# krasserm/perceiver-io

Hardware: NVIDIA H100
Metric: cross_attn_core_tflops (higher is better)
Workload: dtype bf16

## Files before the change

### perceiver_io_b200/csrc/pcv_kvproj.cu

```cuda
#include "pcv_common.cuh"
#include "pcv_sm90.cuh"

#include <algorithm>
#include <cstdlib>

namespace pcv {
namespace {

using namespace sm90;

constexpr int kBM = 128;
constexpr int kBN = 128;
constexpr int kBK = 64;
constexpr int kGemmThreads = 384;
constexpr int kStages = 6;
constexpr int kBoxBytes = 128 * 128;
constexpr int kStageBytes = 2 * kBoxBytes;
constexpr int kSmemBytes = kStages * kStageBytes + 2048 + 1024;

struct GemmParams {
  const float2* stats;
  const float2* col_st;
  void* k_out;
  void* v_out;
  const void* x;
  int64_t x_stride, k_stride, v_stride;
  int64_t rows;
  int n_k, n_total;
  int num_kb;
  int tiles_n;
  int C;
  float eps;
};

struct Fp8Out {
  const float* inv_scale;
  void* vt_out;
  int64_t vt_sb, vt_sh, vt_sc;
  int64_t keys_per_batch;
  int v_dv;
};

struct GemmSmem {
  uint64_t full[kStages], empty[kStages];
  float2 row_st[kBM];
};

template <bool BF16, bool FUSE, int CG, bool F8>
__device__ __forceinline__ void kvproj_body(const CUtensorMap& tx, const CUtensorMap& tw, const GemmParams& p,
                                            const Fp8Out& f8) {
  static_assert(!F8 || CG == 1, "the e4m3 producer runs one CTA per tile");
  using T = typename std::conditional<BF16, __nv_bfloat16, __half>::type;
  extern __shared__ __align__(1024) uint8_t smem_raw[];
  uint8_t* smem = reinterpret_cast<uint8_t*>((reinterpret_cast<uintptr_t>(smem_raw) + 1023) & ~uintptr_t(1023));
  GemmSmem& sh = *reinterpret_cast<GemmSmem*>(smem + kStages * kStageBytes);
  const int wg = threadIdx.x / 128;
  const uint32_t rank = CG == 2 ? cluster_ctarank() : 0u;
  const int64_t cid = blockIdx.x / CG;
  const int n_blk = (int)(cid % p.tiles_n);
  const int64_t m_blk = (cid / p.tiles_n) * CG + rank;
  const int64_t row0 = m_blk * kBM;
  const int col0 = n_blk * kBN;

  if (threadIdx.x == 0) {
    for (int s = 0; s < kStages; ++s) {
      mbar_init(&sh.full[s], 1);
      mbar_init(&sh.empty[s], CG == 2 ? 16 : 8);
    }
    fence_mbar_init();
  }
  if (CG == 2)
    cluster_sync_all();
  else
    __syncthreads();

  if (wg == 0) {
    reg_dealloc<40>();
    if (threadIdx.x == 0) {
      for (int kb = 0; kb < p.num_kb; ++kb) {
// ... 7 lines not shown
        else
          tma_load_2d(smem + s * kStageBytes + kBoxBytes, &tw, &sh.full[s], kb * kBK, col0);
      }
    }
    if (CG == 2) {
      __syncwarp();
      cluster_sync_all();
    }
    return;
  }

  reg_alloc<232>();
  const int cw = wg - 1;
  const int tid = threadIdx.x - 128 * wg;
  const int warp = tid >> 5, lane = tid & 31;
  const int rloc = 64 * cw + 16 * warp + (lane >> 2);
  const int cq = 2 * (lane & 3);
  const uint32_t base = smem_u32(smem);
  const int srow = 64 * cw + (tid >> 1), shalf = tid & 1;
  float x0 = 0.f, s1 = 0.f, s2 = 0.f;
  if (FUSE && row0 + srow < p.rows)
    x0 = Elem<T>::to_f(*(reinterpret_cast<const T*>(p.x) + (row0 + srow) * p.x_stride));

  float acc[64];
  for (int kb = 0; kb < p.num_kb; ++kb) {
    const int s = kb % kStages;
    mbar_wait(&sh.full[s], (kb / kStages) & 1, 12);
    wgmma_fence();
#pragma unroll
    for (int kk = 0; kk < 4; ++kk)
      wgmma_ss<128, BF16>(acc, make_desc(base + s * kStageBytes + cw * 64 * 128 + kk * 32),
                          make_desc(base + s * kStageBytes + kBoxBytes + kk * 32), (kb | kk) != 0);
    wgmma_commit();
    if (FUSE) {
      const uint8_t* line = smem + s * kStageBytes + srow * 128;
#pragma unroll
      for (int ch = 0; ch < 4; ++ch) {
        const int lc = shalf * 4 + ch;
        const uint4 u = *reinterpret_cast<const uint4*>(line + ((lc ^ (srow & 7)) * 16));
        const typename Elem<T>::T2* h2 = reinterpret_cast<const typename Elem<T>::T2*>(&u);
#pragma unroll
        for (int e = 0; e < 4; ++e) {
          const int c = kb * kBK + lc * 8 + 2 * e;
          const float2 f = Elem<T>::to_f2(h2[e]);
          if (c < p.C) {
            const float d = f.x - x0;
            s1 += d;
            s2 = fmaf(d, d, s2);
          }
          if (c + 1 < p.C) {
            const float d = f.y - x0;
            s1 += d;
            s2 = fmaf(d, d, s2);
          }
        }
      }
    }
    wgmma_wait<0>();
    fence_regs(acc);
    if (CG == 2) warp_arrive_pair(&sh.empty[s]);
    else warp_arrive(&sh.empty[s]);
  }

  if (FUSE) {
    s1 += __shfl_xor_sync(0xffffffffu, s1, 1);
    s2 += __shfl_xor_sync(0xffffffffu, s2, 1);
    if (shalf == 0) {
      const float inv_c = 1.f / (float)p.C;
      const float dm = s1 * inv_c;
      const float var = fmaxf(s2 * inv_c - dm * dm, 0.f);
      sh.row_st[srow] = make_float2(x0 + dm, var > 0.f ? rsqrtf(var + p.eps) : 0.f);
    }
    asm volatile("bar.sync %0, 128;" ::"r"(1 + cw) : "memory");
  }

  const float rstd_flat = p.eps > 0.f ? 1.f / sqrtf(p.eps) : -1.f;
#pragma unroll
  for (int r = 0; r < 2; ++r) {
    const int64_t row = row0 + rloc + 8 * r;
    if (row >= p.rows) continue;
    float2 st = make_float2(0.f, 1.f);
    const bool ln = FUSE || p.stats != nullptr;
    if (FUSE) {
      st = sh.row_st[rloc + 8 * r];
    } else if (p.stats != nullptr) {
      st = p.stats[row];
      if (st.y == rstd_flat) st.y = 0.f;
    }
#pragma unroll
    for (int g = 0; g < 16; ++g) {
      const int n = col0 + 8 * g + cq;
      if (n >= p.n_total) continue;
      const float2 c0 = p.col_st[n], c1 = p.col_st[n + 1];
      float a0 = acc[4 * g + 2 * r], a1 = acc[4 * g + 2 * r + 1];
      if (ln) {
        a0 = st.y * (a0 - st.x * c0.x);
        a1 = st.y * (a1 - st.x * c1.x);
      }
      if constexpr (F8) {
        const uint32_t w8 = cvt_e4m3x2((a0 + c0.y) * f8.inv_scale[n], (a1 + c1.y) * f8.inv_scale[n + 1]);
        if (n < p.n_k) {
          *reinterpret_cast<uint16_t*>(reinterpret_cast<uint8_t*>(p.k_out) + row * p.k_stride + n) = (uint16_t)w8;
        } else {
          const int c = n - p.n_k, h = c / f8.v_dv;
          const int64_t b = row / f8.keys_per_batch, m = row - b * f8.keys_per_batch;
          uint8_t* dst = reinterpret_cast<uint8_t*>(f8.vt_out) + b * f8.vt_sb + h * f8.vt_sh +
                         (int64_t)(c - h * f8.v_dv) * f8.vt_sc + m;
          dst[0] = (uint8_t)(w8 & 0xffu);
          dst[f8.vt_sc] = (uint8_t)(w8 >> 8);
        }
      } else {
        const uint32_t w = pack2(a0 + c0.y, a1 + c1.y, BF16);
        if (n < p.n_k)
          *reinterpret_cast<uint32_t*>(reinterpret_cast<T*>(p.k_out) + row * p.k_stride + n) = w;
        else
          *reinterpret_cast<uint32_t*>(reinterpret_cast<T*>(p.v_out) + row * p.v_stride + (n - p.n_k)) = w;
      }
    }
  }
  if (CG == 2) cluster_sync_all();
}

template <bool BF16, bool FUSE, int CG>
__global__ void __launch_bounds__(kGemmThreads, 1)
kvproj_kernel(const __grid_constant__ CUtensorMap tx, const __grid_constant__ CUtensorMap tw, const GemmParams p) {
  kvproj_body<BF16, FUSE, CG, false>(tx, tw, p, Fp8Out{});
}

template <bool BF16, bool FUSE>
__global__ void __launch_bounds__(kGemmThreads, 1)
kvproj_fp8_kernel(const __grid_constant__ CUtensorMap tx, const __grid_constant__ CUtensorMap tw, const GemmParams p,
                  const Fp8Out f8) {
  kvproj_body<BF16, FUSE, 1, true>(tx, tw, p, f8);
}


template <typename T, int NCH>
__global__ void __launch_bounds__(256) ln_stats_reg_kernel(const T* __restrict__ x, int64_t stride_row, int64_t rows,
                                                            float eps, float2* __restrict__ stats) {
  constexpr int C = NCH * 256;
  const int lane = threadIdx.x & 31;
  const int64_t warps = (int64_t)gridDim.x * (blockDim.x >> 5);
  const int64_t w0 = (int64_t)blockIdx.x * (blockDim.x >> 5) + (threadIdx.x >> 5);
  for (int64_t r = w0 * 2; r < rows; r += warps * 2) {
    uint4 u[2][NCH];
#pragma unroll
    for (int k = 0; k < 2; ++k) {
      const bool live = r + k < rows;
      const uint4* xr = reinterpret_cast<const uint4*>(x + (r + k) * stride_row);
#pragma unroll
      for (int i = 0; i < NCH; ++i) u[k][i] = live ? __ldcs(xr + lane + 32 * i) : make_uint4(0, 0, 0, 0);
    }
#pragma unroll
    for (int k = 0; k < 2; ++k) {
      float sum = 0.f;
#pragma unroll
      for (int i = 0; i < NCH; ++i) {
        const typename Elem<T>::T2* h = reinterpret_cast<const typename Elem<T>::T2*>(&u[k][i]);
#pragma unroll
        for (int j = 0; j < 4; ++j) {
          const float2 f = Elem<T>::to_f2(h[j]);
          sum += f.x + f.y;
        }
      }
      const float mean = warp_sum(sum) / (float)C;
      float sq = 0.f;
#pragma unroll
      for (int i = 0; i < NCH; ++i) {
// ... 69 lines not shown
    const int blocks = (int)std::min<int64_t>((p.rows + 15) / 16, 132 * 8);
#define PCV_LN_CASE(N)                                                                               \
  case N:                                                                                            \
    ln_stats_reg_kernel<T, N><<<blocks, 256, 0, stream>>>(x, p.x_stride_row, p.rows, p.eps, st);     \
    break;
    switch (p.C / 256) {
      PCV_LN_CASE(1) PCV_LN_CASE(2) PCV_LN_CASE(3) PCV_LN_CASE(4) PCV_LN_CASE(5) PCV_LN_CASE(6) PCV_LN_CASE(7)
      PCV_LN_CASE(8)
    }
#undef PCV_LN_CASE
  } else {
    const int blocks = (int)std::min<int64_t>((p.rows + 7) / 8, 132 * 8);
    ln_stats_kernel<T><<<blocks, 256, 0, stream>>>(x, p.x_stride_row, p.rows, p.C, p.eps, st);
  }
  PCV_CHECK_CUDA(cudaGetLastError());
  count_launch();
  return PCV_OK;
}

template <bool BF16, bool FUSE, int CG, bool F8 = false>
int launch_gemm(const CUtensorMap& tx, const CUtensorMap& tw, const GemmParams& gp, cudaStream_t stream,
                const Fp8Out& f8 = Fp8Out{}) {
  const int64_t m_blocks = (gp.rows + kBM * CG - 1) / (kBM * CG) * CG;
  const int64_t tiles = m_blocks * gp.tiles_n;
  PCV_REQUIRE(tiles <= 0x7fffffff, PCV_ERR_UNSUPPORTED, "kv_project: %lld tiles exceed the grid limit", (long long)tiles);
  prof_mark_begin(stream);
  int rc;
  if constexpr (F8)
    rc = launch_kernel(kvproj_fp8_kernel<BF16, FUSE>, dim3((unsigned)tiles), kGemmThreads, kSmemBytes, 0, stream, tx, tw,
                       gp, f8);
  else
    rc = launch_kernel(kvproj_kernel<BF16, FUSE, CG>, dim3((unsigned)tiles), kGemmThreads, kSmemBytes, CG, stream,
                       tx, tw, gp);
  prof_mark_end(stream);
  return rc;
}

}

int launch_ln_stats(const pcv_ln_stats_params& p, cudaStream_t stream) {
  PCV_REQUIRE(p.x != nullptr && p.stats != nullptr, PCV_ERR_INVALID, "ln_stats: NULL pointer");
  PCV_REQUIRE(p.rows >= 0 && p.C >= 1, PCV_ERR_INVALID, "ln_stats: rows=%lld C=%d", (long long)p.rows, p.C);
  PCV_REQUIRE(p.dtype == PCV_BF16 || p.dtype == PCV_F16, PCV_ERR_INVALID, "ln_stats: dtype must be bf16/fp16");
  if (p.rows == 0) return PCV_OK;
  return p.dtype == PCV_BF16 ? launch_ln_stats_t<__nv_bfloat16>(p, stream) : launch_ln_stats_t<__half>(p, stream);
}

bool kv_project_supported(const pcv_kvproj_params& p, const char** why) {
  auto fail = [&](const char* w) {
    *why = w;
    return false;
  };
  if (p.dtype != PCV_BF16 && p.dtype != PCV_F16) return fail("dtype must be bf16 or fp16");
  if (p.C < 8 || (p.C % 8)) return fail("input channels must be a multiple of 8 (16-byte TMA strides)");
  if (p.n_k < 0 || p.n_v < 0 || p.n_k + p.n_v < 1) return fail("no output columns");
  if ((p.n_k % 64) != 0) return fail("K width must be a multiple of 64");
  if ((p.n_v % 8) != 0) return fail("V width must be a multiple of 8");
  if (!al16(p.x) || !al16(p.w) || (p.n_k && !al16(p.k_out)) || (p.n_v && !al16(p.v_out)))
    return fail("x / w / k_out / v_out must be 16-byte aligned");
  if ((p.x_stride_row % 8) || (p.k_stride_row % 8) || (p.v_stride_row % 8)) return fail("row strides must be multiples of 8 elements");
  if (p.rows < 1 || p.rows > (int64_t)0x7fffff00) return fail("row count out of range");
  if (p.cta_group < 0 || p.cta_group > 2) return fail("cta_group must be 0, 1 or 2");
  if (const char* w = device_problem()) return fail(w);
  return true;
}

// ... 57 lines not shown
  if (fuse)
    return bf ? launch_gemm<true, true, 1, true>(tx, tw, gp, stream, f8) : launch_gemm<false, true, 1, true>(tx, tw, gp, stream, f8);
  return bf ? launch_gemm<true, false, 1, true>(tx, tw, gp, stream, f8) : launch_gemm<false, false, 1, true>(tx, tw, gp, stream, f8);
}

int launch_kv_project(const pcv_kvproj_params& p, cudaStream_t stream) {
  const char* why = "";
  PCV_REQUIRE(p.x && p.w && p.col_st, PCV_ERR_INVALID, "kv_project: NULL pointer");
  PCV_REQUIRE(kv_project_supported(p, &why), PCV_ERR_UNSUPPORTED, "kv_project: %s", why);
  const int n_total = p.n_k + p.n_v;
  GemmParams gp{};
  gp.stats = reinterpret_cast<const float2*>(p.row_stats);
  gp.col_st = reinterpret_cast<const float2*>(p.col_st);
  gp.k_out = p.k_out;
  gp.v_out = p.v_out;
  gp.x = p.x;
  gp.x_stride = p.x_stride_row;
  gp.k_stride = p.k_stride_row;
  gp.v_stride = p.v_stride_row;
  gp.rows = p.rows;
  gp.n_k = p.n_k;
  gp.n_total = n_total;
  gp.num_kb = (p.C + kBK - 1) / kBK;
  gp.tiles_n = (n_total + kBN - 1) / kBN;
  gp.C = p.C;
  gp.eps = p.ln_eps;
  const bool fuse = p.row_stats == nullptr && p.ln_eps > 0.f;

  int rc = attach_wait_diag(&g_wait_diag);
  if (rc != PCV_OK) return rc;
  CUtensorMap tx, tw;
  rc = make_tmap_2d(&tx, p.x, p.dtype, p.C, p.rows, p.x_stride_row, kBM);
  if (rc != PCV_OK) return rc;
  const int cg = p.cta_group == 2 ? 2 : 1;
  rc = make_tmap_2d(&tw, p.w, p.dtype, p.C, n_total, p.C, kBN / cg);
  if (rc != PCV_OK) return rc;
  const bool bf = p.dtype == PCV_BF16;
#define PCV_GEMM_CASE(G)                                                                                   \
  if (fuse) return bf ? launch_gemm<true, true, G>(tx, tw, gp, stream) : launch_gemm<false, true, G>(tx, tw, gp, stream); \
  return bf ? launch_gemm<true, false, G>(tx, tw, gp, stream) : launch_gemm<false, false, G>(tx, tw, gp, stream);
  if (cg == 2) {
    PCV_GEMM_CASE(2)
  }
  PCV_GEMM_CASE(1)
#undef PCV_GEMM_CASE
}

}
```

### perceiver_io_b200/csrc/pcv_sm90.cuh

```cuda
#pragma once

#include <cstdint>
#include <utility>
#include <cuda.h>
#include <cuda_runtime.h>

#include "pcv_common.cuh"

namespace pcv {
namespace sm90 {

__device__ __forceinline__ uint32_t smem_u32(const void* p) {
  return static_cast<uint32_t>(__cvta_generic_to_shared(p));
}

__device__ __forceinline__ void mbar_init(uint64_t* bar, uint32_t count) {
  asm volatile("mbarrier.init.shared::cta.b64 [%0], %1;" ::"r"(smem_u32(bar)), "r"(count) : "memory");
}
__device__ __forceinline__ void fence_mbar_init() {
  asm volatile("fence.mbarrier_init.release.cluster;" ::: "memory");
}
__device__ __forceinline__ void fence_proxy_async_smem() {
  asm volatile("fence.proxy.async.shared::cta;" ::: "memory");
}
// ... 51 lines not shown
  }
}

__device__ __forceinline__ void warp_arrive(uint64_t* bar) {
  __syncwarp();
  if ((threadIdx.x & 31) == 0) mbar_arrive(bar);
}

template <int ID, int THREADS>
__device__ __forceinline__ void named_bar_sync() {
  asm volatile("bar.sync %0, %1;" ::"n"(ID), "n"(THREADS) : "memory");
}
template <int ID, int THREADS>
__device__ __forceinline__ void named_bar_arrive() {
  asm volatile("bar.arrive %0, %1;" ::"n"(ID), "n"(THREADS) : "memory");
}

__device__ __forceinline__ void tma_load_4d(void* smem_dst, const void* tmap, uint64_t* bar, int c0, int c1,
                                            int c2, int c3) {
  asm volatile(
      "cp.async.bulk.tensor.4d.shared::cluster.global.mbarrier::complete_tx::bytes [%0], [%1, {%3, %4, %5, %6}], "
      "[%2];" ::"r"(smem_u32(smem_dst)),
      "l"(reinterpret_cast<uint64_t>(tmap)), "r"(smem_u32(bar)), "r"(c0), "r"(c1), "r"(c2), "r"(c3)
      : "memory");
}
__device__ __forceinline__ void tma_load_2d(void* smem_dst, const void* tmap, uint64_t* bar, int c0, int c1) {
  asm volatile(
      "cp.async.bulk.tensor.2d.shared::cluster.global.mbarrier::complete_tx::bytes [%0], [%1, {%3, %4}], [%2];" ::"r"(
          smem_u32(smem_dst)),
      "l"(reinterpret_cast<uint64_t>(tmap)), "r"(smem_u32(bar)), "r"(c0), "r"(c1)
      : "memory");
}

__device__ __forceinline__ uint32_t cluster_ctarank() {
  uint32_t r;
  asm volatile("mov.u32 %0, %%cluster_ctarank;" : "=r"(r));
  return r;
}
__device__ __forceinline__ void cluster_sync_all() {
  asm volatile("barrier.cluster.arrive.release.aligned;\n\tbarrier.cluster.wait.acquire.aligned;" ::: "memory");
}
__device__ __forceinline__ void mbar_arrive_cta(uint64_t* bar, uint32_t cta) {
  uint32_t remote;
  asm volatile("mapa.shared::cluster.u32 %0, %1, %2;" : "=r"(remote) : "r"(smem_u32(bar)), "r"(cta));
  asm volatile("mbarrier.arrive.release.cluster.shared::cluster.b64 _, [%0];" ::"r"(remote) : "memory");
}
__device__ __forceinline__ void warp_arrive_pair(uint64_t* bar) {
  __syncwarp();
  if ((threadIdx.x & 31) == 0) {
    mbar_arrive_cta(bar, 0);
    mbar_arrive_cta(bar, 1);
  }
}
__device__ __forceinline__ void wg_arrive(uint64_t* bar) {
  if ((threadIdx.x & 127) == 0) mbar_arrive(bar);
}
__device__ __forceinline__ void wg_arrive_pair(uint64_t* bar) {
  const uint32_t t = threadIdx.x & 127;
  if (t == 0) mbar_arrive(bar);
  else if (t == 32) mbar_arrive_cta(bar, cluster_ctarank() ^ 1u);
}
__device__ __forceinline__ void tma_load_4d_mc(void* smem_dst, const void* tmap, uint64_t* bar, int c0, int c1, int c2,
                                               int c3, uint16_t mask) {
  asm volatile(
      "cp.async.bulk.tensor.4d.shared::cluster.global.mbarrier::complete_tx::bytes.multicast::cluster [%0], [%1, {%3, "
      "%4, %5, %6}], [%2], %7;" ::"r"(smem_u32(smem_dst)),
// ... 107 lines not shown
      "{%0, %1, %2, %3, %4, %5, %6, %7, %8, %9, %10, %11, %12, %13, %14, %15, %16, %17, %18, %19, %20, %21, %22, %23, %24, %25, %26, %27, %28, %29, %30, %31, %32, %33, %34, %35, %36, %37, %38, %39, %40, %41, %42, %43, %44, %45, %46, %47, %48, %49, %50, %51, %52, %53, %54, %55, %56, %57, %58, %59, %60, %61, %62, %63}, %64, %65, p, 1, 1, 0, 0;\n\t}"
      : "+f"(d[0]), "+f"(d[1]), "+f"(d[2]), "+f"(d[3]), "+f"(d[4]), "+f"(d[5]), "+f"(d[6]), "+f"(d[7]), "+f"(d[8]), "+f"(d[9]), "+f"(d[10]), "+f"(d[11]), "+f"(d[12]), "+f"(d[13]), "+f"(d[14]), "+f"(d[15]), "+f"(d[16]), "+f"(d[17]), "+f"(d[18]), "+f"(d[19]), "+f"(d[20]), "+f"(d[21]), "+f"(d[22]), "+f"(d[23]), "+f"(d[24]), "+f"(d[25]), "+f"(d[26]), "+f"(d[27]), "+f"(d[28]), "+f"(d[29]), "+f"(d[30]), "+f"(d[31]), "+f"(d[32]), "+f"(d[33]), "+f"(d[34]), "+f"(d[35]), "+f"(d[36]), "+f"(d[37]), "+f"(d[38]), "+f"(d[39]), "+f"(d[40]), "+f"(d[41]), "+f"(d[42]), "+f"(d[43]), "+f"(d[44]), "+f"(d[45]), "+f"(d[46]), "+f"(d[47]), "+f"(d[48]), "+f"(d[49]), "+f"(d[50]), "+f"(d[51]), "+f"(d[52]), "+f"(d[53]), "+f"(d[54]), "+f"(d[55]), "+f"(d[56]), "+f"(d[57]), "+f"(d[58]), "+f"(d[59]), "+f"(d[60]), "+f"(d[61]), "+f"(d[62]), "+f"(d[63])
      : "l"(a), "l"(b), "r"(scale_d));
}

template <>
__device__ __forceinline__ void wgmma_rs<64, false>(float (&d)[32], const uint32_t (&a)[4], uint64_t b) {
  asm volatile(
      "{\n\t.reg .pred p;\n\tsetp.ne.b32 p, 1, 0;\n\t"
      "wgmma.mma_async.sync.aligned.m64n64k16.f32.f16.f16 "
      "{%0, %1, %2, %3, %4, %5, %6, %7, %8, %9, %10, %11, %12, %13, %14, %15, %16, %17, %18, %19, %20, %21, %22, %23, %24, %25, %26, %27, %28, %29, %30, %31}, {%32, %33, %34, %35}, %36, p, 1, 1, 1;\n\t}"
      : "+f"(d[0]), "+f"(d[1]), "+f"(d[2]), "+f"(d[3]), "+f"(d[4]), "+f"(d[5]), "+f"(d[6]), "+f"(d[7]), "+f"(d[8]), "+f"(d[9]), "+f"(d[10]), "+f"(d[11]), "+f"(d[12]), "+f"(d[13]), "+f"(d[14]), "+f"(d[15]), "+f"(d[16]), "+f"(d[17]), "+f"(d[18]), "+f"(d[19]), "+f"(d[20]), "+f"(d[21]), "+f"(d[22]), "+f"(d[23]), "+f"(d[24]), "+f"(d[25]), "+f"(d[26]), "+f"(d[27]), "+f"(d[28]), "+f"(d[29]), "+f"(d[30]), "+f"(d[31])
      : "r"(a[0]), "r"(a[1]), "r"(a[2]), "r"(a[3]), "l"(b));
}

template <>
__device__ __forceinline__ void wgmma_rs<128, true>(float (&d)[64], const uint32_t (&a)[4], uint64_t b) {
  asm volatile(
      "{\n\t.reg .pred p;\n\tsetp.ne.b32 p, 1, 0;\n\t"
      "wgmma.mma_async.sync.aligned.m64n128k16.f32.bf16.bf16 "
      "{%0, %1, %2, %3, %4, %5, %6, %7, %8, %9, %10, %11, %12, %13, %14, %15, %16, %17, %18, %19, %20, %21, %22, %23, %24, %25, %26, %27, %28, %29, %30, %31, %32, %33, %34, %35, %36, %37, %38, %39, %40, %41, %42, %43, %44, %45, %46, %47, %48, %49, %50, %51, %52, %53, %54, %55, %56, %57, %58, %59, %60, %61, %62, %63}, {%64, %65, %66, %67}, %68, p, 1, 1, 1;\n\t}"
      : "+f"(d[0]), "+f"(d[1]), "+f"(d[2]), "+f"(d[3]), "+f"(d[4]), "+f"(d[5]), "+f"(d[6]), "+f"(d[7]), "+f"(d[8]), "+f"(d[9]), "+f"(d[10]), "+f"(d[11]), "+f"(d[12]), "+f"(d[13]), "+f"(d[14]), "+f"(d[15]), "+f"(d[16]), "+f"(d[17]), "+f"(d[18]), "+f"(d[19]), "+f"(d[20]), "+f"(d[21]), "+f"(d[22]), "+f"(d[23]), "+f"(d[24]), "+f"(d[25]), "+f"(d[26]), "+f"(d[27]), "+f"(d[28]), "+f"(d[29]), "+f"(d[30]), "+f"(d[31]), "+f"(d[32]), "+f"(d[33]), "+f"(d[34]), "+f"(d[35]), "+f"(d[36]), "+f"(d[37]), "+f"(d[38]), "+f"(d[39]), "+f"(d[40]), "+f"(d[41]), "+f"(d[42]), "+f"(d[43]), "+f"(d[44]), "+f"(d[45]), "+f"(d[46]), "+f"(d[47]), "+f"(d[48]), "+f"(d[49]), "+f"(d[50]), "+f"(d[51]), "+f"(d[52]), "+f"(d[53]), "+f"(d[54]), "+f"(d[55]), "+f"(d[56]), "+f"(d[57]), "+f"(d[58]), "+f"(d[59]), "+f"(d[60]), "+f"(d[61]), "+f"(d[62]), "+f"(d[63])
      : "r"(a[0]), "r"(a[1]), "r"(a[2]), "r"(a[3]), "l"(b));
}

template <>
__device__ __forceinline__ void wgmma_rs<128, false>(float (&d)[64], const uint32_t (&a)[4], uint64_t b) {
  asm volatile(
      "{\n\t.reg .pred p;\n\tsetp.ne.b32 p, 1, 0;\n\t"
      "wgmma.mma_async.sync.aligned.m64n128k16.f32.f16.f16 "
      "{%0, %1, %2, %3, %4, %5, %6, %7, %8, %9, %10, %11, %12, %13, %14, %15, %16, %17, %18, %19, %20, %21, %22, %23, %24, %25, %26, %27, %28, %29, %30, %31, %32, %33, %34, %35, %36, %37, %38, %39, %40, %41, %42, %43, %44, %45, %46, %47, %48, %49, %50, %51, %52, %53, %54, %55, %56, %57, %58, %59, %60, %61, %62, %63}, {%64, %65, %66, %67}, %68, p, 1, 1, 1;\n\t}"
      : "+f"(d[0]), "+f"(d[1]), "+f"(d[2]), "+f"(d[3]), "+f"(d[4]), "+f"(d[5]), "+f"(d[6]), "+f"(d[7]), "+f"(d[8]), "+f"(d[9]), "+f"(d[10]), "+f"(d[11]), "+f"(d[12]), "+f"(d[13]), "+f"(d[14]), "+f"(d[15]), "+f"(d[16]), "+f"(d[17]), "+f"(d[18]), "+f"(d[19]), "+f"(d[20]), "+f"(d[21]), "+f"(d[22]), "+f"(d[23]), "+f"(d[24]), "+f"(d[25]), "+f"(d[26]), "+f"(d[27]), "+f"(d[28]), "+f"(d[29]), "+f"(d[30]), "+f"(d[31]), "+f"(d[32]), "+f"(d[33]), "+f"(d[34]), "+f"(d[35]), "+f"(d[36]), "+f"(d[37]), "+f"(d[38]), "+f"(d[39]), "+f"(d[40]), "+f"(d[41]), "+f"(d[42]), "+f"(d[43]), "+f"(d[44]), "+f"(d[45]), "+f"(d[46]), "+f"(d[47]), "+f"(d[48]), "+f"(d[49]), "+f"(d[50]), "+f"(d[51]), "+f"(d[52]), "+f"(d[53]), "+f"(d[54]), "+f"(d[55]), "+f"(d[56]), "+f"(d[57]), "+f"(d[58]), "+f"(d[59]), "+f"(d[60]), "+f"(d[61]), "+f"(d[62]), "+f"(d[63])
      : "r"(a[0]), "r"(a[1]), "r"(a[2]), "r"(a[3]), "l"(b));
}

template <bool BF16>
__device__ __forceinline__ void wgmma_ss_bmn_n128(float (&d)[64], uint64_t a, uint64_t b, int scale_d) {
  if constexpr (BF16)
    asm volatile(
        "{\n\t.reg .pred p;\n\tsetp.ne.b32 p, %66, 0;\n\t"
        "wgmma.mma_async.sync.aligned.m64n128k16.f32.bf16.bf16 "
        "{%0, %1, %2, %3, %4, %5, %6, %7, %8, %9, %10, %11, %12, %13, %14, %15, %16, %17, %18, %19, %20, %21, %22, %23, %24, %25, %26, %27, %28, %29, %30, %31, %32, %33, %34, %35, %36, %37, %38, %39, %40, %41, %42, %43, %44, %45, %46, %47, %48, %49, %50, %51, %52, %53, %54, %55, %56, %57, %58, %59, %60, %61, %62, %63}, %64, %65, p, 1, 1, 0, 1;\n\t}"
        : "+f"(d[0]), "+f"(d[1]), "+f"(d[2]), "+f"(d[3]), "+f"(d[4]), "+f"(d[5]), "+f"(d[6]), "+f"(d[7]), "+f"(d[8]), "+f"(d[9]), "+f"(d[10]), "+f"(d[11]), "+f"(d[12]), "+f"(d[13]), "+f"(d[14]), "+f"(d[15]), "+f"(d[16]), "+f"(d[17]), "+f"(d[18]), "+f"(d[19]), "+f"(d[20]), "+f"(d[21]), "+f"(d[22]), "+f"(d[23]), "+f"(d[24]), "+f"(d[25]), "+f"(d[26]), "+f"(d[27]), "+f"(d[28]), "+f"(d[29]), "+f"(d[30]), "+f"(d[31]), "+f"(d[32]), "+f"(d[33]), "+f"(d[34]), "+f"(d[35]), "+f"(d[36]), "+f"(d[37]), "+f"(d[38]), "+f"(d[39]), "+f"(d[40]), "+f"(d[41]), "+f"(d[42]), "+f"(d[43]), "+f"(d[44]), "+f"(d[45]), "+f"(d[46]), "+f"(d[47]), "+f"(d[48]), "+f"(d[49]), "+f"(d[50]), "+f"(d[51]), "+f"(d[52]), "+f"(d[53]), "+f"(d[54]), "+f"(d[55]), "+f"(d[56]), "+f"(d[57]), "+f"(d[58]), "+f"(d[59]), "+f"(d[60]), "+f"(d[61]), "+f"(d[62]), "+f"(d[63])
        : "l"(a), "l"(b), "r"(scale_d));
  else
    asm volatile(
        "{\n\t.reg .pred p;\n\tsetp.ne.b32 p, %66, 0;\n\t"
        "wgmma.mma_async.sync.aligned.m64n128k16.f32.f16.f16 "
        "{%0, %1, %2, %3, %4, %5, %6, %7, %8, %9, %10, %11, %12, %13, %14, %15, %16, %17, %18, %19, %20, %21, %22, %23, %24, %25, %26, %27, %28, %29, %30, %31, %32, %33, %34, %35, %36, %37, %38, %39, %40, %41, %42, %43, %44, %45, %46, %47, %48, %49, %50, %51, %52, %53, %54, %55, %56, %57, %58, %59, %60, %61, %62, %63}, %64, %65, p, 1, 1, 0, 1;\n\t}"
        : "+f"(d[0]), "+f"(d[1]), "+f"(d[2]), "+f"(d[3]), "+f"(d[4]), "+f"(d[5]), "+f"(d[6]), "+f"(d[7]), "+f"(d[8]), "+f"(d[9]), "+f"(d[10]), "+f"(d[11]), "+f"(d[12]), "+f"(d[13]), "+f"(d[14]), "+f"(d[15]), "+f"(d[16]), "+f"(d[17]), "+f"(d[18]), "+f"(d[19]), "+f"(d[20]), "+f"(d[21]), "+f"(d[22]), "+f"(d[23]), "+f"(d[24]), "+f"(d[25]), "+f"(d[26]), "+f"(d[27]), "+f"(d[28]), "+f"(d[29]), "+f"(d[30]), "+f"(d[31]), "+f"(d[32]), "+f"(d[33]), "+f"(d[34]), "+f"(d[35]), "+f"(d[36]), "+f"(d[37]), "+f"(d[38]), "+f"(d[39]), "+f"(d[40]), "+f"(d[41]), "+f"(d[42]), "+f"(d[43]), "+f"(d[44]), "+f"(d[45]), "+f"(d[46]), "+f"(d[47]), "+f"(d[48]), "+f"(d[49]), "+f"(d[50]), "+f"(d[51]), "+f"(d[52]), "+f"(d[53]), "+f"(d[54]), "+f"(d[55]), "+f"(d[56]), "+f"(d[57]), "+f"(d[58]), "+f"(d[59]), "+f"(d[60]), "+f"(d[61]), "+f"(d[62]), "+f"(d[63])
        : "l"(a), "l"(b), "r"(scale_d));
}

__device__ __forceinline__ void ldsm_x4_trans(uint32_t (&r)[4], uint32_t addr) {
  asm volatile("ldmatrix.sync.aligned.m8n8.x4.trans.shared.b16 {%0, %1, %2, %3}, [%4];"
               : "=r"(r[0]), "=r"(r[1]), "=r"(r[2]), "=r"(r[3])
               : "r"(addr)
               : "memory");
}

__device__ __forceinline__ void wgmma_ss_e4m3_n128(float (&d)[64], uint64_t a, uint64_t b, int scale_d) {
  asm volatile(
      "{\n\t.reg .pred p;\n\tsetp.ne.b32 p, %66, 0;\n\t"
      "wgmma.mma_async.sync.aligned.m64n128k32.f32.e4m3.e4m3 "
      "{%0, %1, %2, %3, %4, %5, %6, %7, %8, %9, %10, %11, %12, %13, %14, %15, %16, %17, %18, %19, %20, %21, %22, %23, %24, %25, %26, %27, %28, %29, %30, %31, %32, %33, %34, %35, %36, %37, %38, %39, %40, %41, %42, %43, %44, %45, %46, %47, %48, %49, %50, %51, %52, %53, %54, %55, %56, %57, %58, %59, %60, %61, %62, %63}, %64, %65, p, 1, 1;\n\t}"
      : "+f"(d[0]), "+f"(d[1]), "+f"(d[2]), "+f"(d[3]), "+f"(d[4]), "+f"(d[5]), "+f"(d[6]), "+f"(d[7]), "+f"(d[8]), "+f"(d[9]), "+f"(d[10]), "+f"(d[11]), "+f"(d[12]), "+f"(d[13]), "+f"(d[14]), "+f"(d[15]), "+f"(d[16]), "+f"(d[17]), "+f"(d[18]), "+f"(d[19]), "+f"(d[20]), "+f"(d[21]), "+f"(d[22]), "+f"(d[23]), "+f"(d[24]), "+f"(d[25]), "+f"(d[26]), "+f"(d[27]), "+f"(d[28]), "+f"(d[29]), "+f"(d[30]), "+f"(d[31]), "+f"(d[32]), "+f"(d[33]), "+f"(d[34]), "+f"(d[35]), "+f"(d[36]), "+f"(d[37]), "+f"(d[38]), "+f"(d[39]), "+f"(d[40]), "+f"(d[41]), "+f"(d[42]), "+f"(d[43]), "+f"(d[44]), "+f"(d[45]), "+f"(d[46]), "+f"(d[47]), "+f"(d[48]), "+f"(d[49]), "+f"(d[50]), "+f"(d[51]), "+f"(d[52]), "+f"(d[53]), "+f"(d[54]), "+f"(d[55]), "+f"(d[56]), "+f"(d[57]), "+f"(d[58]), "+f"(d[59]), "+f"(d[60]), "+f"(d[61]), "+f"(d[62]), "+f"(d[63])
// ... 48 lines not shown
```

Measured before the change: 589.9.

## Add persistent 128x256 KV-projection GEMM with TMA-store epilogue

Adds a persistent warp-specialized kernel, used when cta_group is 0 and there are at least as many tiles as SMs. It uses 128x256 tiles with m64n256 wgmma and keeps one wgmma group in flight across k-blocks. Output goes through swizzled shared-memory staging and TMA bulk stores, aiming to cut launch and tail overhead and to overlap the epilogue with the next tile's loads. In exchange it uses 128 fp32 accumulators per thread, has only 3 pipeline stages, and does not handle the fp8 path. The workload metric is cross-attention core TFLOPS, so the kv-projection may not dominate it.

```diff
diff --git a/perceiver_io_b200/csrc/pcv_kvproj.cu b/perceiver_io_b200/csrc/pcv_kvproj.cu
--- a/perceiver_io_b200/csrc/pcv_kvproj.cu
+++ b/perceiver_io_b200/csrc/pcv_kvproj.cu
@@ -45,6 +45,64 @@
   uint64_t full[kStages], empty[kStages];
   float2 row_st[kBM];
 };
+
+template <typename T>
+__device__ __forceinline__ void stats_accumulate(const uint8_t* line, int srow, int shalf, int kb, const GemmParams& p,
+                                                 float x0, float& s1, float& s2) {
+#pragma unroll
+  for (int ch = 0; ch < 4; ++ch) {
+    const int lc = shalf * 4 + ch;
+    const uint4 u = *reinterpret_cast<const uint4*>(line + ((lc ^ (srow & 7)) * 16));
+    const typename Elem<T>::T2* h2 = reinterpret_cast<const typename Elem<T>::T2*>(&u);
+#pragma unroll
+    for (int e = 0; e < 4; ++e) {
+      const int c = kb * kBK + lc * 8 + 2 * e;
+      const float2 f = Elem<T>::to_f2(h2[e]);
+      if (c < p.C) {
+        const float d = f.x - x0;
+        s1 += d;
+        s2 = fmaf(d, d, s2);
+      }
+      if (c + 1 < p.C) {
+        const float d = f.y - x0;
+        s1 += d;
+        s2 = fmaf(d, d, s2);
+      }
+    }
+  }
+}
+
+__device__ __forceinline__ void stats_finish(float x0, float s1, float s2, int srow, int shalf, const GemmParams& p,
+                                             float2* row_st) {
+  s1 += __shfl_xor_sync(0xffffffffu, s1, 1);
+  s2 += __shfl_xor_sync(0xffffffffu, s2, 1);
+  if (shalf == 0) {
+    const float inv_c = 1.f / (float)p.C;
+    const float dm = s1 * inv_c;
+    const float var = fmaxf(s2 * inv_c - dm * dm, 0.f);
+    row_st[srow] = make_float2(x0 + dm, var > 0.f ? rsqrtf(var + p.eps) : 0.f);
+  }
+}
+
+template <bool FUSE>
+__device__ __forceinline__ float2 epilogue_stats(const GemmParams& p, const float2* row_st, int rloc, int64_t row,
+                                                 float rstd_flat) {
+  float2 st = make_float2(0.f, 1.f);
+  if (FUSE) {
+    st = row_st[rloc];
+  } else if (p.stats != nullptr) {
+    st = p.stats[row];
+    if (st.y == rstd_flat) st.y = 0.f;
+  }
+  return st;
+}
+
+__device__ __forceinline__ void epilogue_ln(float& a0, float& a1, float2 st, float2 c0, float2 c1, bool ln) {
+  if (ln) {
+    a0 = st.y * (a0 - st.x * c0.x);
+    a1 = st.y * (a1 - st.x * c1.x);
+  }
+}
 
 template <bool BF16, bool FUSE, int CG, bool F8>
 __device__ __forceinline__ void kvproj_body(const CUtensorMap& tx, const CUtensorMap& tw, const GemmParams& p,
@@ -118,30 +176,7 @@
       wgmma_ss<128, BF16>(acc, make_desc(base + s * kStageBytes + cw * 64 * 128 + kk * 32),
                           make_desc(base + s * kStageBytes + kBoxBytes + kk * 32), (kb | kk) != 0);
     wgmma_commit();
-    if (FUSE) {
-      const uint8_t* line = smem + s * kStageBytes + srow * 128;
-#pragma unroll
-      for (int ch = 0; ch < 4; ++ch) {
-        const int lc = shalf * 4 + ch;
-        const uint4 u = *reinterpret_cast<const uint4*>(line + ((lc ^ (srow & 7)) * 16));
-        const typename Elem<T>::T2* h2 = reinterpret_cast<const typename Elem<T>::T2*>(&u);
-#pragma unroll
-        for (int e = 0; e < 4; ++e) {
-          const int c = kb * kBK + lc * 8 + 2 * e;
-          const float2 f = Elem<T>::to_f2(h2[e]);
-          if (c < p.C) {
-            const float d = f.x - x0;
-            s1 += d;
-            s2 = fmaf(d, d, s2);
-          }
-          if (c + 1 < p.C) {
-            const float d = f.y - x0;
-            s1 += d;
-            s2 = fmaf(d, d, s2);
-          }
-        }
-      }
-    }
+    if (FUSE) stats_accumulate<T>(smem + s * kStageBytes + srow * 128, srow, shalf, kb, p, x0, s1, s2);
     wgmma_wait<0>();
     fence_regs(acc);
     if (CG == 2) warp_arrive_pair(&sh.empty[s]);
@@ -149,14 +184,7 @@
   }
 
   if (FUSE) {
-    s1 += __shfl_xor_sync(0xffffffffu, s1, 1);
-    s2 += __shfl_xor_sync(0xffffffffu, s2, 1);
-    if (shalf == 0) {
-      const float inv_c = 1.f / (float)p.C;
-      const float dm = s1 * inv_c;
-      const float var = fmaxf(s2 * inv_c - dm * dm, 0.f);
-      sh.row_st[srow] = make_float2(x0 + dm, var > 0.f ? rsqrtf(var + p.eps) : 0.f);
-    }
+    stats_finish(x0, s1, s2, srow, shalf, p, sh.row_st);
     asm volatile("bar.sync %0, 128;" ::"r"(1 + cw) : "memory");
   }
 
@@ -165,24 +193,15 @@
   for (int r = 0; r < 2; ++r) {
     const int64_t row = row0 + rloc + 8 * r;
     if (row >= p.rows) continue;
-    float2 st = make_float2(0.f, 1.f);
     const bool ln = FUSE || p.stats != nullptr;
-    if (FUSE) {
-      st = sh.row_st[rloc + 8 * r];
-    } else if (p.stats != nullptr) {
-      st = p.stats[row];
-      if (st.y == rstd_flat) st.y = 0.f;
-    }
+    const float2 st = epilogue_stats<FUSE>(p, sh.row_st, rloc + 8 * r, row, rstd_flat);
 #pragma unroll
     for (int g = 0; g < 16; ++g) {
       const int n = col0 + 8 * g + cq;
       if (n >= p.n_total) continue;
       const float2 c0 = p.col_st[n], c1 = p.col_st[n + 1];
       float a0 = acc[4 * g + 2 * r], a1 = acc[4 * g + 2 * r + 1];
-      if (ln) {
-        a0 = st.y * (a0 - st.x * c0.x);
-        a1 = st.y * (a1 - st.x * c1.x);
-      }
+      epilogue_ln(a0, a1, st, c0, c1, ln);
       if constexpr (F8) {
         const uint32_t w8 = cvt_e4m3x2((a0 + c0.y) * f8.inv_scale[n], (a1 + c1.y) * f8.inv_scale[n + 1]);
         if (n < p.n_k) {
@@ -220,6 +239,154 @@
   kvproj_body<BF16, FUSE, 1, true>(tx, tw, p, f8);
 }
 
+constexpr int kPBN = 256;
+constexpr int kPStages = 3;
+constexpr int kPStageBytes = kBoxBytes + 2 * kBoxBytes;
+constexpr int kPOutBoxBytes = 64 * 128;
+constexpr int kPOutBytes = 4 * kPOutBoxBytes;
+constexpr int kPSmemBytes = kPStages * kPStageBytes + 2 * kPOutBytes + 2048 + 1024;
+
+struct PersistSmem {
+  uint64_t full[kPStages], empty[kPStages];
+  float2 row_st[kBM];
+};
+
+template <bool BF16, bool FUSE>
+__global__ void __launch_bounds__(kGemmThreads, 1)
+kvproj_persistent_kernel(const __grid_constant__ CUtensorMap tx, const __grid_constant__ CUtensorMap tw,
+                         const __grid_constant__ CUtensorMap tk, const __grid_constant__ CUtensorMap tv,
+                         const GemmParams p) {
+  using T = typename std::conditional<BF16, __nv_bfloat16, __half>::type;
+  extern __shared__ __align__(1024) uint8_t smem_raw[];
+  uint8_t* smem = reinterpret_cast<uint8_t*>((reinterpret_cast<uintptr_t>(smem_raw) + 1023) & ~uintptr_t(1023));
+  uint8_t* out_smem = smem + kPStages * kPStageBytes;
+  PersistSmem& sh = *reinterpret_cast<PersistSmem*>(out_smem + 2 * kPOutBytes);
+  const int wg = threadIdx.x / 128;
+  const int64_t tiles = (p.rows + kBM - 1) / kBM * p.tiles_n;
+
+  if (threadIdx.x == 0) {
+    for (int s = 0; s < kPStages; ++s) {
+      mbar_init(&sh.full[s], 1);
+      mbar_init(&sh.empty[s], 8);
+    }
+    fence_mbar_init();
+  }
+  __syncthreads();
+
+  if (wg == 0) {
+    reg_dealloc<40>();
+    if (threadIdx.x == 0) {
+      int s = 0;
+      uint32_t phase = 0;
+      for (int64_t t = blockIdx.x; t < tiles; t += gridDim.x) {
+        const int row0 = (int)(t / p.tiles_n) * kBM;
+        const int col0 = (int)(t % p.tiles_n) * kPBN;
+        const bool w1 = col0 + kBN < p.n_total;
+        for (int kb = 0; kb < p.num_kb; ++kb) {
+          mbar_wait(&sh.empty[s], phase ^ 1, 13);
+          uint8_t* st = smem + s * kPStageBytes;
+          mbar_arrive_expect_tx(&sh.full[s], w1 ? kPStageBytes : 2 * kBoxBytes);
+          tma_load_2d(st, &tx, &sh.full[s], kb * kBK, row0);
+          tma_load_2d(st + kBoxBytes, &tw, &sh.full[s], kb * kBK, col0);
+          if (w1) tma_load_2d(st + 2 * kBoxBytes, &tw, &sh.full[s], kb * kBK, col0 + kBN);
+          if (++s == kPStages) {
+            s = 0;
+            phase ^= 1;
+          }
+        }
+      }
+    }
+    return;
+  }
+
+  reg_alloc<232>();
+  const int cw = wg - 1;
+  const int tid = threadIdx.x - 128 * wg;
+  const int warp = tid >> 5, lane = tid & 31;
+  const int rw = 16 * warp + (lane >> 2);
+  const int cq = 2 * (lane & 3);
+  const uint32_t base = smem_u32(smem);
+  uint8_t* out = out_smem + cw * kPOutBytes;
+  const int srow = 64 * cw + (tid >> 1), shalf = tid & 1;
+  const float rstd_flat = p.eps > 0.f ? 1.f / sqrtf(p.eps) : -1.f;
+  const bool ln = FUSE || p.stats != nullptr;
+  int s = 0;
+  uint32_t phase = 0;
+  float acc[128];
+  for (int64_t t = blockIdx.x; t < tiles; t += gridDim.x) {
+    const int64_t row0 = (t / p.tiles_n) * kBM;
+    const int col0 = (int)(t % p.tiles_n) * kPBN;
+    float x0 = 0.f, s1 = 0.f, s2 = 0.f;
+    if (FUSE && row0 + srow < p.rows)
+      x0 = Elem<T>::to_f(*(reinterpret_cast<const T*>(p.x) + (row0 + srow) * p.x_stride));
+
+    int prev = 0;
+    for (int kb = 0; kb < p.num_kb; ++kb) {
+      mbar_wait(&sh.full[s], phase, 14);
+      wgmma_fence();
+#pragma unroll
+      for (int kk = 0; kk < 4; ++kk)
+        wgmma_ss<256, BF16>(acc, make_desc(base + s * kPStageBytes + cw * 64 * 128 + kk * 32),
+                            make_desc(base + s * kPStageBytes + kBoxBytes + kk * 32), (kb | kk) != 0);
+      wgmma_commit();
+      if (FUSE) stats_accumulate<T>(smem + s * kPStageBytes + srow * 128, srow, shalf, kb, p, x0, s1, s2);
+      wgmma_wait<1>();
+      if (kb > 0) warp_arrive(&sh.empty[prev]);
+      prev = s;
+      if (++s == kPStages) {
+        s = 0;
+        phase ^= 1;
+      }
+    }
+    wgmma_wait<0>();
+    fence_regs(acc);
+    warp_arrive(&sh.empty[prev]);
+
+    if (FUSE) stats_finish(x0, s1, s2, srow, shalf, p, sh.row_st);
+    if (tid == 0) bulk_wait_read<0>();
+    asm volatile("bar.sync %0, 128;" ::"r"(1 + cw) : "memory");
+
+    float2 st[2];
+    bool live[2];
+#pragma unroll
+    for (int r = 0; r < 2; ++r) {
+      const int64_t row = row0 + 64 * cw + rw + 8 * r;
+      live[r] = row < p.rows;
+      st[r] = live[r] ? epilogue_stats<FUSE>(p, sh.row_st, 64 * cw + rw + 8 * r, row, rstd_flat) : make_float2(0.f, 1.f);
+    }
+#pragma unroll
+    for (int g = 0; g < 32; ++g) {
+      const int n = col0 + 8 * g + cq;
+      if (n >= p.n_total) continue;
+      const float2 c0 = p.col_st[n], c1 = p.col_st[n + 1];
+#pragma unroll
+      for (int r = 0; r < 2; ++r) {
+        if (!live[r]) continue;
+        float a0 = acc[4 * g + 2 * r], a1 = acc[4 * g + 2 * r + 1];
+        epilogue_ln(a0, a1, st[r], c0, c1, ln);
+        const int rl = rw + 8 * r;
+        *reinterpret_cast<uint32_t*>(out + (g >> 3) * kPOutBoxBytes + rl * 128 + (((g & 7) ^ (rl & 7)) << 4) + 2 * cq) =
+            pack2(a0 + c0.y, a1 + c1.y, BF16);
+      }
+    }
+    fence_proxy_async_smem();
+    asm volatile("bar.sync %0, 128;" ::"r"(1 + cw) : "memory");
+    const int64_t r0 = row0 + 64 * cw;
+    if (tid == 0 && r0 < p.rows) {
+#pragma unroll
+      for (int b = 0; b < 4; ++b) {
+        const int c = col0 + 64 * b;
+        if (c >= p.n_total) break;
+        if (c < p.n_k)
+          tma_store_2d(&tk, out + b * kPOutBoxBytes, c, (int)r0);
+        else
+          tma_store_2d(&tv, out + b * kPOutBoxBytes, c - p.n_k, (int)r0);
+      }
+      bulk_commit();
+    }
+  }
+  if (tid == 0) bulk_wait<0>();
+}
 
 template <typename T, int NCH>
 __global__ void __launch_bounds__(256) ln_stats_reg_kernel(const T* __restrict__ x, int64_t stride_row, int64_t rows,
@@ -355,6 +522,25 @@
   else
     rc = launch_kernel(kvproj_kernel<BF16, FUSE, CG>, dim3((unsigned)tiles), kGemmThreads, kSmemBytes, CG, stream,
                        tx, tw, gp);
+  prof_mark_end(stream);
+  return rc;
+}
+
+int64_t persistent_tiles(int64_t rows, int n_total) { return (rows + kBM - 1) / kBM * ((n_total + kPBN - 1) / kPBN); }
+
+int sm_count() {
+  int dev = 0, sms = 0;
+  PCV_CHECK_CUDA(cudaGetDevice(&dev));
+  PCV_CHECK_CUDA(cudaDeviceGetAttribute(&sms, cudaDevAttrMultiProcessorCount, dev));
+  return sms;
+}
+
+template <bool BF16, bool FUSE>
+int launch_persistent(const CUtensorMap& tx, const CUtensorMap& tw, const CUtensorMap& tk, const CUtensorMap& tv,
+                      const GemmParams& gp, int grid, cudaStream_t stream) {
+  prof_mark_begin(stream);
+  const int rc = launch_kernel(kvproj_persistent_kernel<BF16, FUSE>, dim3((unsigned)grid), kGemmThreads, kPSmemBytes, 0,
+                               stream, tx, tw, tk, tv, gp);
   prof_mark_end(stream);
   return rc;
 }
@@ -478,10 +664,28 @@
   CUtensorMap tx, tw;
   rc = make_tmap_2d(&tx, p.x, p.dtype, p.C, p.rows, p.x_stride_row, kBM);
   if (rc != PCV_OK) return rc;
+  const bool bf = p.dtype == PCV_BF16;
+  if (p.cta_group == 0) {
+    const int64_t tiles = persistent_tiles(p.rows, n_total);
+    const int sms = sm_count();
+    if (sms <= 0) return PCV_ERR_CUDA;
+    if (tiles >= sms) {
+      rc = make_tmap_2d(&tw, p.w, p.dtype, p.C, n_total, p.C, kBN);
+      if (rc != PCV_OK) return rc;
+      CUtensorMap tk{}, tv{};
+      if (p.n_k > 0 && (rc = make_tmap_2d(&tk, p.k_out, p.dtype, p.n_k, p.rows, p.k_stride_row, 64)) != PCV_OK) return rc;
+      if (p.n_v > 0 && (rc = make_tmap_2d(&tv, p.v_out, p.dtype, p.n_v, p.rows, p.v_stride_row, 64)) != PCV_OK) return rc;
+      gp.tiles_n = (n_total + kPBN - 1) / kPBN;
+      if (fuse)
+        return bf ? launch_persistent<true, true>(tx, tw, tk, tv, gp, sms, stream)
+                  : launch_persistent<false, true>(tx, tw, tk, tv, gp, sms, stream);
+      return bf ? launch_persistent<true, false>(tx, tw, tk, tv, gp, sms, stream)
+                : launch_persistent<false, false>(tx, tw, tk, tv, gp, sms, stream);
+    }
+  }
   const int cg = p.cta_group == 2 ? 2 : 1;
   rc = make_tmap_2d(&tw, p.w, p.dtype, p.C, n_total, p.C, kBN / cg);
   if (rc != PCV_OK) return rc;
-  const bool bf = p.dtype == PCV_BF16;
 #define PCV_GEMM_CASE(G)                                                                                   \
   if (fuse) return bf ? launch_gemm<true, true, G>(tx, tw, gp, stream) : launch_gemm<false, true, G>(tx, tw, gp, stream); \
   return bf ? launch_gemm<true, false, G>(tx, tw, gp, stream) : launch_gemm<false, false, G>(tx, tw, gp, stream);
diff --git a/perceiver_io_b200/csrc/pcv_sm90.cuh b/perceiver_io_b200/csrc/pcv_sm90.cuh
--- a/perceiver_io_b200/csrc/pcv_sm90.cuh
+++ b/perceiver_io_b200/csrc/pcv_sm90.cuh
@@ -107,6 +107,22 @@
       : "memory");
 }
 
+__device__ __forceinline__ void tma_store_2d(const void* tmap, const void* smem_src, int c0, int c1) {
+  asm volatile("cp.async.bulk.tensor.2d.global.shared::cta.bulk_group [%0, {%2, %3}], [%1];" ::"l"(
+                   reinterpret_cast<uint64_t>(tmap)),
+               "r"(smem_u32(smem_src)), "r"(c0), "r"(c1)
+               : "memory");
+}
+__device__ __forceinline__ void bulk_commit() { asm volatile("cp.async.bulk.commit_group;" ::: "memory"); }
+template <int N>
+__device__ __forceinline__ void bulk_wait_read() {
+  asm volatile("cp.async.bulk.wait_group.read %0;" ::"n"(N) : "memory");
+}
+template <int N>
+__device__ __forceinline__ void bulk_wait() {
+  asm volatile("cp.async.bulk.wait_group %0;" ::"n"(N) : "memory");
+}
+
 __device__ __forceinline__ uint32_t cluster_ctarank() {
   uint32_t r;
   asm volatile("mov.u32 %0, %%cluster_ctarank;" : "=r"(r));
@@ -280,6 +296,26 @@
       "{%0, %1, %2, %3, %4, %5, %6, %7, %8, %9, %10, %11, %12, %13, %14, %15, %16, %17, %18, %19, %20, %21, %22, %23, %24, %25, %26, %27, %28, %29, %30, %31, %32, %33, %34, %35, %36, %37, %38, %39, %40, %41, %42, %43, %44, %45, %46, %47, %48, %49, %50, %51, %52, %53, %54, %55, %56, %57, %58, %59, %60, %61, %62, %63}, {%64, %65, %66, %67}, %68, p, 1, 1, 1;\n\t}"
       : "+f"(d[0]), "+f"(d[1]), "+f"(d[2]), "+f"(d[3]), "+f"(d[4]), "+f"(d[5]), "+f"(d[6]), "+f"(d[7]), "+f"(d[8]), "+f"(d[9]), "+f"(d[10]), "+f"(d[11]), "+f"(d[12]), "+f"(d[13]), "+f"(d[14]), "+f"(d[15]), "+f"(d[16]), "+f"(d[17]), "+f"(d[18]), "+f"(d[19]), "+f"(d[20]), "+f"(d[21]), "+f"(d[22]), "+f"(d[23]), "+f"(d[24]), "+f"(d[25]), "+f"(d[26]), "+f"(d[27]), "+f"(d[28]), "+f"(d[29]), "+f"(d[30]), "+f"(d[31]), "+f"(d[32]), "+f"(d[33]), "+f"(d[34]), "+f"(d[35]), "+f"(d[36]), "+f"(d[37]), "+f"(d[38]), "+f"(d[39]), "+f"(d[40]), "+f"(d[41]), "+f"(d[42]), "+f"(d[43]), "+f"(d[44]), "+f"(d[45]), "+f"(d[46]), "+f"(d[47]), "+f"(d[48]), "+f"(d[49]), "+f"(d[50]), "+f"(d[51]), "+f"(d[52]), "+f"(d[53]), "+f"(d[54]), "+f"(d[55]), "+f"(d[56]), "+f"(d[57]), "+f"(d[58]), "+f"(d[59]), "+f"(d[60]), "+f"(d[61]), "+f"(d[62]), "+f"(d[63])
       : "r"(a[0]), "r"(a[1]), "r"(a[2]), "r"(a[3]), "l"(b));
+}
+
+template <>
+__device__ __forceinline__ void wgmma_ss<256, true>(float (&d)[128], uint64_t a, uint64_t b, int scale_d) {
+  asm volatile(
+      "{\n\t.reg .pred p;\n\tsetp.ne.b32 p, %130, 0;\n\t"
+      "wgmma.mma_async.sync.aligned.m64n256k16.f32.bf16.bf16 "
+      "{%0, %1, %2, %3, %4, %5, %6, %7, %8, %9, %10, %11, %12, %13, %14, %15, %16, %17, %18, %19, %20, %21, %22, %23, %24, %25, %26, %27, %28, %29, %30, %31, %32, %33, %34, %35, %36, %37, %38, %39, %40, %41, %42, %43, %44, %45, %46, %47, %48, %49, %50, %51, %52, %53, %54, %55, %56, %57, %58, %59, %60, %61, %62, %63, %64, %65, %66, %67, %68, %69, %70, %71, %72, %73, %74, %75, %76, %77, %78, %79, %80, %81, %82, %83, %84, %85, %86, %87, %88, %89, %90, %91, %92, %93, %94, %95, %96, %97, %98, %99, %100, %101, %102, %103, %104, %105, %106, %107, %108, %109, %110, %111, %112, %113, %114, %115, %116, %117, %118, %119, %120, %121, %122, %123, %124, %125, %126, %127}, %128, %129, p, 1, 1, 0, 0;\n\t}"
+      : "+f"(d[0]), "+f"(d[1]), "+f"(d[2]), "+f"(d[3]), "+f"(d[4]), "+f"(d[5]), "+f"(d[6]), "+f"(d[7]), "+f"(d[8]), "+f"(d[9]), "+f"(d[10]), "+f"(d[11]), "+f"(d[12]), "+f"(d[13]), "+f"(d[14]), "+f"(d[15]), "+f"(d[16]), "+f"(d[17]), "+f"(d[18]), "+f"(d[19]), "+f"(d[20]), "+f"(d[21]), "+f"(d[22]), "+f"(d[23]), "+f"(d[24]), "+f"(d[25]), "+f"(d[26]), "+f"(d[27]), "+f"(d[28]), "+f"(d[29]), "+f"(d[30]), "+f"(d[31]), "+f"(d[32]), "+f"(d[33]), "+f"(d[34]), "+f"(d[35]), "+f"(d[36]), "+f"(d[37]), "+f"(d[38]), "+f"(d[39]), "+f"(d[40]), "+f"(d[41]), "+f"(d[42]), "+f"(d[43]), "+f"(d[44]), "+f"(d[45]), "+f"(d[46]), "+f"(d[47]), "+f"(d[48]), "+f"(d[49]), "+f"(d[50]), "+f"(d[51]), "+f"(d[52]), "+f"(d[53]), "+f"(d[54]), "+f"(d[55]), "+f"(d[56]), "+f"(d[57]), "+f"(d[58]), "+f"(d[59]), "+f"(d[60]), "+f"(d[61]), "+f"(d[62]), "+f"(d[63]), "+f"(d[64]), "+f"(d[65]), "+f"(d[66]), "+f"(d[67]), "+f"(d[68]), "+f"(d[69]), "+f"(d[70]), "+f"(d[71]), "+f"(d[72]), "+f"(d[73]), "+f"(d[74]), "+f"(d[75]), "+f"(d[76]), "+f"(d[77]), "+f"(d[78]), "+f"(d[79]), "+f"(d[80]), "+f"(d[81]), "+f"(d[82]), "+f"(d[83]), "+f"(d[84]), "+f"(d[85]), "+f"(d[86]), "+f"(d[87]), "+f"(d[88]), "+f"(d[89]), "+f"(d[90]), "+f"(d[91]), "+f"(d[92]), "+f"(d[93]), "+f"(d[94]), "+f"(d[95]), "+f"(d[96]), "+f"(d[97]), "+f"(d[98]), "+f"(d[99]), "+f"(d[100]), "+f"(d[101]), "+f"(d[102]), "+f"(d[103]), "+f"(d[104]), "+f"(d[105]), "+f"(d[106]), "+f"(d[107]), "+f"(d[108]), "+f"(d[109]), "+f"(d[110]), "+f"(d[111]), "+f"(d[112]), "+f"(d[113]), "+f"(d[114]), "+f"(d[115]), "+f"(d[116]), "+f"(d[117]), "+f"(d[118]), "+f"(d[119]), "+f"(d[120]), "+f"(d[121]), "+f"(d[122]), "+f"(d[123]), "+f"(d[124]), "+f"(d[125]), "+f"(d[126]), "+f"(d[127])
+      : "l"(a), "l"(b), "r"(scale_d));
+}
+
+template <>
+__device__ __forceinline__ void wgmma_ss<256, false>(float (&d)[128], uint64_t a, uint64_t b, int scale_d) {
+  asm volatile(
+      "{\n\t.reg .pred p;\n\tsetp.ne.b32 p, %130, 0;\n\t"
+      "wgmma.mma_async.sync.aligned.m64n256k16.f32.f16.f16 "
+      "{%0, %1, %2, %3, %4, %5, %6, %7, %8, %9, %10, %11, %12, %13, %14, %15, %16, %17, %18, %19, %20, %21, %22, %23, %24, %25, %26, %27, %28, %29, %30, %31, %32, %33, %34, %35, %36, %37, %38, %39, %40, %41, %42, %43, %44, %45, %46, %47, %48, %49, %50, %51, %52, %53, %54, %55, %56, %57, %58, %59, %60, %61, %62, %63, %64, %65, %66, %67, %68, %69, %70, %71, %72, %73, %74, %75, %76, %77, %78, %79, %80, %81, %82, %83, %84, %85, %86, %87, %88, %89, %90, %91, %92, %93, %94, %95, %96, %97, %98, %99, %100, %101, %102, %103, %104, %105, %106, %107, %108, %109, %110, %111, %112, %113, %114, %115, %116, %117, %118, %119, %120, %121, %122, %123, %124, %125, %126, %127}, %128, %129, p, 1, 1, 0, 0;\n\t}"
+      : "+f"(d[0]), "+f"(d[1]), "+f"(d[2]), "+f"(d[3]), "+f"(d[4]), "+f"(d[5]), "+f"(d[6]), "+f"(d[7]), "+f"(d[8]), "+f"(d[9]), "+f"(d[10]), "+f"(d[11]), "+f"(d[12]), "+f"(d[13]), "+f"(d[14]), "+f"(d[15]), "+f"(d[16]), "+f"(d[17]), "+f"(d[18]), "+f"(d[19]), "+f"(d[20]), "+f"(d[21]), "+f"(d[22]), "+f"(d[23]), "+f"(d[24]), "+f"(d[25]), "+f"(d[26]), "+f"(d[27]), "+f"(d[28]), "+f"(d[29]), "+f"(d[30]), "+f"(d[31]), "+f"(d[32]), "+f"(d[33]), "+f"(d[34]), "+f"(d[35]), "+f"(d[36]), "+f"(d[37]), "+f"(d[38]), "+f"(d[39]), "+f"(d[40]), "+f"(d[41]), "+f"(d[42]), "+f"(d[43]), "+f"(d[44]), "+f"(d[45]), "+f"(d[46]), "+f"(d[47]), "+f"(d[48]), "+f"(d[49]), "+f"(d[50]), "+f"(d[51]), "+f"(d[52]), "+f"(d[53]), "+f"(d[54]), "+f"(d[55]), "+f"(d[56]), "+f"(d[57]), "+f"(d[58]), "+f"(d[59]), "+f"(d[60]), "+f"(d[61]), "+f"(d[62]), "+f"(d[63]), "+f"(d[64]), "+f"(d[65]), "+f"(d[66]), "+f"(d[67]), "+f"(d[68]), "+f"(d[69]), "+f"(d[70]), "+f"(d[71]), "+f"(d[72]), "+f"(d[73]), "+f"(d[74]), "+f"(d[75]), "+f"(d[76]), "+f"(d[77]), "+f"(d[78]), "+f"(d[79]), "+f"(d[80]), "+f"(d[81]), "+f"(d[82]), "+f"(d[83]), "+f"(d[84]), "+f"(d[85]), "+f"(d[86]), "+f"(d[87]), "+f"(d[88]), "+f"(d[89]), "+f"(d[90]), "+f"(d[91]), "+f"(d[92]), "+f"(d[93]), "+f"(d[94]), "+f"(d[95]), "+f"(d[96]), "+f"(d[97]), "+f"(d[98]), "+f"(d[99]), "+f"(d[100]), "+f"(d[101]), "+f"(d[102]), "+f"(d[103]), "+f"(d[104]), "+f"(d[105]), "+f"(d[106]), "+f"(d[107]), "+f"(d[108]), "+f"(d[109]), "+f"(d[110]), "+f"(d[111]), "+f"(d[112]), "+f"(d[113]), "+f"(d[114]), "+f"(d[115]), "+f"(d[116]), "+f"(d[117]), "+f"(d[118]), "+f"(d[119]), "+f"(d[120]), "+f"(d[121]), "+f"(d[122]), "+f"(d[123]), "+f"(d[124]), "+f"(d[125]), "+f"(d[126]), "+f"(d[127])
+      : "l"(a), "l"(b), "r"(scale_d));
 }
 
 template <bool BF16>
```

Measured after the change: 604.9, median of 6. +2.5%, better.
